# zhipeng-wei/Image-to-Video-I2V-attack

Measured on AMD Instinct MI355X. Metric: adversarial frames/sec (10-step I2V, ResNet-50 layer3, 32x224^2 clips), higher is better.
Workload: dtype f32

## Files before the change

image-to-video-i2v-attack_amd/csrc/i2v_conv_tile.h:

```cpp
#pragma once
#include "i2v_be.h"

#ifndef I2V_PROBE_T
struct I2VNoProbe {
    __device__ __forceinline__ void entry() {}
    __device__ __forceinline__ void loop_begin() {}
    __device__ __forceinline__ void loop_end(int ) {}
    __device__ __forceinline__ void exit(int ) {}
};
#define I2V_PROBE_T I2VNoProbe
#endif

#ifndef I2V_PRIO_LEVELS
#define I2V_PRIO_LEVELS 3
#endif
#ifndef I2V_DEEP
#define I2V_DEEP 1
#endif
#ifndef I2V_DEEP_STAGES
#define I2V_DEEP_STAGES 3
#endif
#ifndef I2V_BF3_STAGES
#define I2V_BF3_STAGES 2
#endif
#ifndef I2V_SMALL_WPE
#define I2V_SMALL_WPE 7
#endif
#ifndef I2V_PREF_WPE
#define I2V_PREF_WPE 6
#endif
#ifndef I2V_MID_WPE
#define I2V_MID_WPE 5
#endif
#ifndef I2V_TALL_WPE
#define I2V_TALL_WPE 6
#endif
#ifndef I2V_BIG_WPE
#define I2V_BIG_WPE 3
#endif

static constexpr int conv_waves_per_simd(int BD, int BP, bool PREF, bool hi, int MODE = 0) {
    return (BD == 64 && BP == 64) ? (PREF ? (I2V_DEEP && MODE == 1 && I2V_DEEP_STAGES > 3 ? 4  : I2V_PREF_WPE) : I2V_SMALL_WPE) : (BD == 128 && BP == 64) ? I2V_TALL_WPE : (BD == 32 && BP == 256) ? 4  : BD * BP == 8192 ? I2V_MID_WPE : BD * BP == 16384 ? I2V_BIG_WPE : (hi ? 8 : 1);
}
#define I2V_CONV_WPE __attribute__((amdgpu_waves_per_eu(conv_waves_per_simd(BD, BP, PREF, false, MODE), conv_waves_per_simd(BD, BP, PREF, true, MODE))))
static constexpr bool conv_deep(int MODE, bool PREF) { return I2V_DEEP && PREF && MODE == 1; }
template <int BD, int BP, int WD, bool MF16, int NST = 2, int CPB = 1, int BF3 = 0>
constexpr int conv_lds_floats() {
    constexpr int stage = NST * CPB * (I2V_KC * BP + (BF3 == 2 ? 0 : BF3 ? ((BD / 32) * 3 + 3) / 4 * 4 * 256 : I2V_KC * BD)), epi = WD * (MF16 ? 16 : 32) * BP;
    return stage > epi ? stage : epi;
}

template <int HWM>
constexpr int conv_halo_lds_floats() {
    constexpr int stage = 2 * I2V_KC * (64 + 64 + 2 * HWM + 2), epi = 64 * 64;
    return stage > epi ? stage : epi;
}

template <int BD, int BP, int WD, bool PREF, bool MF16, bool FUSE, typename PT>
__device__ __forceinline__ void conv_vec_rows(const PT& p, const int i, const int cd0, const int64_t px0, const float (*const Cs)[BP], const int t,
                                              const float4* const pre0, const unsigned* const pregw, float* const mid) {
    constexpr int FR = MF16 ? 16 : 32;
    const int lane = t & 63;
    const int HWg = p.Hg * p.Wg, HoWo = p.Ho * p.Wo;
    const int64_t P = (int64_t)p.N * HWg;
    (void)pre0; (void)pregw; (void)mid;
#ifdef I2V_NT_ALL
    const bool nt_store = true;
#else
    const bool nt_store = p.cfg > 0 && ((p.cfg - 1) & 128);
#endif
    constexpr int C4 = BP / 4, RSTEP = 1024 / BP, NQ = WD * FR / RSTEP;
    const int c4 = t % C4, rbase = t / C4;
    const int64_t pp = px0 + (int64_t)c4 * 4;
    const bool pok = pp < P;
    const int64_t n = pok ? fastdiv((unsigned)pp, p.dv_hw_m, p.dv_hw_s) : 0;
    const int64_t poff = pp - n * HWg;
    #pragma unroll
    for (int q = 0; q < NQ; ++q) {
        const int row = rbase + q * RSTEP;
        const int cd = cd0 + (row / FR) * (BD / WD) + i * FR + (row % FR);
        const bool valid = pok && cd < p.Cd;
        float4 v = make_float4(0.f, 0.f, 0.f, 0.f);
        if (valid) {
        v = *reinterpret_cast<const float4*>(&Cs[row][c4 * 4]);
        const int64_t o = (int64_t)cd * HoWo + poff;
        if (p.gate_scale) {
            const float4 m = *reinterpret_cast<const float4*>(p.mask + n * p.mask_nstride + o);
            const float gs = p.gate_scale[cd], gt = p.gate_shift[cd];
            if (!(fmaf(m.x, gs, gt) > 0.f)) v.x = 0.f;
            if (!(fmaf(m.y, gs, gt) > 0.f)) v.y = 0.f;
            if (!(fmaf(m.z, gs, gt) > 0.f)) v.z = 0.f;
            if (!(fmaf(m.w, gs, gt) > 0.f)) v.w = 0.f;
        }
        if (p.shift) { const float sh = p.shift[cd]; v.x += sh; v.y += sh; v.z += sh; v.w += sh; }
        if (PREF) {
            v.x += pre0[q].x; v.y += pre0[q].y; v.z += pre0[q].z; v.w += pre0[q].w;
        } else {
            if (p.add0 && p.add0_stride == 1) {
                const float4 a = *reinterpret_cast<const float4*>(p.add0 + n * p.add0_nstride + o);
                v.x += a.x; v.y += a.y; v.z += a.z; v.w += a.w;
            } else if (p.add0) {
                const int oh = (int)fastdiv((unsigned)poff, p.dv_wo_m, p.dv_wo_s), ow = (int)(poff - (int64_t)oh * p.Wo);
                if (!(oh & 1) && (oh >> 1) < p.add0_H) {
                    const float2 a = *reinterpret_cast<const float2*>(
                        p.add0 + n * p.add0_nstride + (int64_t)cd * p.add0_H * p.add0_W + (oh >> 1) * p.add0_W + (ow >> 1));
                    v.x += a.x; v.z += a.y;
                }
            }
        }
        if (p.add1) {
            const float4 a = *reinterpret_cast<const float4*>(p.add1 + n * p.add1_nstride + o);
            v.x += a.x; v.y += a.y; v.z += a.z; v.w += a.w;
        }
        if (p.relu) { v.x = fmaxf(v.x, 0.f); v.y = fmaxf(v.y, 0.f); v.z = fmaxf(v.z, 0.f); v.w = fmaxf(v.w, 0.f); }
        if (p.gate) {
            const unsigned w = PREF ? pregw[q] : p.gate[(int64_t)cd * p.gate_stride + ((p.gate_pix0 + pp) >> 5)];
            const unsigned g = w >> ((unsigned)(p.gate_pix0 + pp) & 31u);
            if (!(g & 1u)) v.x = 0.f;
            if (!(g & 2u)) v.y = 0.f;
            if (!(g & 4u)) v.z = 0.f;
            if (!(g & 8u)) v.w = 0.f;
        } else if (p.mask && !p.gate_scale) {
            const float4 m = *reinterpret_cast<const float4*>(p.mask + n * p.mask_nstride + o);
            if (!(m.x > 0.f)) v.x = 0.f;
            if (!(m.y > 0.f)) v.y = 0.f;
            if (!(m.z > 0.f)) v.z = 0.f;
            if (!(m.w > 0.f)) v.w = 0.f;
        }
        if constexpr (!FUSE) {
            if (nt_store) { typedef float nt4 __attribute__((ext_vector_type(4))); const nt4 w4 = {v.x, v.y, v.z, v.w};
                            __builtin_nontemporal_store(w4, reinterpret_cast<nt4*>(p.dst + n * p.dst_nstride + o)); }
            else *reinterpret_cast<float4*>(p.dst + n * p.dst_nstride + o) = v;
        }
        }
        if constexpr (FUSE)
            *reinterpret_cast<float4*>(mid + (cd - cd0) * BP + c4 * 4) = v;
        if (p.gate_out) {
            unsigned nib = valid ? ((v.x > 0.f ? 1u : 0u) | (v.y > 0.f ? 2u : 0u) | (v.z > 0.f ? 4u : 0u) | (v.w > 0.f ? 8u : 0u)) : 0u;
            nib <<= 4 * (lane & 7);
            nib |= (unsigned)__builtin_amdgcn_update_dpp(0, (int)nib, 0xB1, 0xF, 0xF, true);
            nib |= (unsigned)__builtin_amdgcn_update_dpp(0, (int)nib, 0x4E, 0xF, 0xF, true);
            nib |= (unsigned)__builtin_amdgcn_update_dpp(0, (int)nib, 0x141, 0xF, 0xF, true);
            if (valid && (lane & 7) == 0)
                p.gate_out[(int64_t)cd * p.gate_out_stride + ((p.gate_out_pix0 + pp) >> 5)] = nib;
        }
    }
}

#define I2V_FROW(r) (MF16 ? 4 * lk + (r) : ((r) & 3) + 8 * ((r) >> 2) + 4 * lk)
template <int BP, int WP, bool MF16, int TP, typename ACC>
__device__ __forceinline__ void conv_acc_to_rows(ACC (&acc)[TP], float (*const Cs)[BP]) {
    constexpr int FR = MF16 ? 16 : 32, NR = MF16 ? 4 : 16;
    const int lane = threadIdx.x & 63, wave = threadIdx.x >> 6;
    const int wd = wave / WP, wpx = wave % WP;
    const int l31 = MF16 ? (lane & 15) : (lane & 31), lk = MF16 ? (lane >> 4) : (lane >> 5);
    __syncthreads();
#pragma unroll
    for (int j = 0; j < TP; ++j)
#pragma unroll
        for (int r = 0; r < NR; ++r)
            Cs[wd * FR + I2V_FROW(r)][wpx * (BP / WP) + j * FR + l31] = acc[j][r];
    __syncthreads();
}
template <int BD, int BP, int WD, int WP, bool PREF, bool MF16, bool FUSE, typename ACC, typename PT>
__device__ __forceinline__ void conv_vec_epilogue(const PT& p, ACC (&acc)[BD / WD / (MF16 ? 16 : 32)][BP / WP / (MF16 ? 16 : 32)], const int cd0,
                                                  const int64_t px0, float* const smem, const float4* const pre0, const unsigned* const pregw,
                                                  float* const mid) {
    constexpr int FR = MF16 ? 16 : 32, TD = BD / WD / FR;
    const int t = threadIdx.x;
    float (*Cs)[BP] = reinterpret_cast<float (*)[BP]>(smem);
#pragma unroll
    for (int i = 0; i < TD; ++i) {
        conv_acc_to_rows<BP, WP, MF16>(acc[i], Cs);
        conv_vec_rows<BD, BP, WD, PREF, MF16, FUSE>(p, i, cd0, px0, Cs, t, pre0, pregw, mid);
    }
}
#undef I2V_FROW

__device__ __forceinline__ int conv_xcd_lid(const int bid, const int nwg) {
    const int q8 = nwg >> 3, r8 = nwg & 7, xcd = bid & 7;
    return (xcd < r8 ? xcd * (q8 + 1) : r8 * (q8 + 1) + (xcd - r8) * q8) + (bid >> 3);
}

template <int BD, int BP, int WD, int WP, int MODE, bool PREF, bool PRE = false, bool VID = false, bool MF16 = false, int HWM = 0, int CPB = 1, int FUSE = 0, int BF3 = 0>
__device__ __forceinline__ void conv_tile_loop(const I2VConvParams& p, const int cd0, const int64_t px0, const int nwg, float* const smem, I2V_PROBE_T& probe,
                                               const int probe_slot, const int prio_arg,
                                               typename std::conditional<MF16, f32x4, f32x16>::type (&acc)[BD / WD / (MF16 ? 16 : 32)][BP / WP / (MF16 ? 16 : 32)],
                                               float4 (&pre0)[PREF ? WD * (MF16 ? 16 : 32) / (1024 / BP) : 1], unsigned (&pregw)[PREF ? WD * (MF16 ? 16 : 32) / (1024 / BP) : 1]) {
#if defined(__HIP_DEVICE_COMPILE__)
    constexpr int KC = I2V_KC;
    constexpr int FR = MF16 ? 16 : 32;
    constexpr int NR = MF16 ? 4 : 16;
    constexpr int TD = BD / WD / FR, TP = BP / WP / FR;
    static_assert(!(MF16 && (PRE || PREF)), "no pre-activation / prefetch variants of the 16x16 tile");
    constexpr bool DEEP = conv_deep(MODE, PREF) || (BF3 == 1 && I2V_BF3_STAGES > 2) || BF3 == 3;
    constexpr int NST = BF3 == 3 ? 3 : BF3 == 1 ? I2V_BF3_STAGES : DEEP ? I2V_DEEP_STAGES : 2, AHEAD = NST - 1;
    constexpr bool HALO = MODE == 5;
    constexpr int HS = HALO ? BP + 2 * HWM + 2 : 1, HQ = (HS + 63) / 64;
    static_assert(!HALO || (HWM > 0 && BD == 64 && BP == 64 && !PREF && !PRE && !VID && !MF16), "halo staging: the plain 64x64 image tile only");
    static_assert(CPB == 1 || (!HALO && !DEEP && !PREF && !PRE && MODE != 4 && MODE != 0), "several chunks per barrier: the plain pointwise / tap-uniform loops only");
    constexpr int KB = CPB * KC;
    static_assert(!BF3 || (!MF16 && !PRE && !PREF && !HALO && (MODE == 1 || MODE == 2) && FUSE == 0 && BD % 32 == 0), "split-bf16 K loop: the plain pointwise / tap-uniform tiles");
    constexpr int AF = BF3 == 2 ? 0 : BF3 ? CPB * (((BD / 32) * 3 + 3) / 4 * 4) * 256 : KB * BD;
    float (*As)[KB][BD] = reinterpret_cast<float (*)[KB][BD]>(smem);
    float* const As3 = smem;
    float (*Bs)[KB][BP] = reinterpret_cast<float (*)[KB][BP]>(smem + NST * AF);

    const int t = threadIdx.x, lane = t & 63, wave = t >> 6;
    const int wd = wave / WP, wpx = wave % WP;

    const int HWg = p.Hg * p.Wg;
    const int64_t P = (int64_t)p.N * HWg;

    constexpr bool PW = MODE == 1;
    constexpr bool QUAD = MODE == 4;
    typedef __attribute__((address_space(3))) void* lds_ptr_t;
    constexpr unsigned OOB = 0x80000000u;
    const int wv = __builtin_amdgcn_readfirstlane(wave);
    const __amdgpu_buffer_rsrc_t rs_w = BF3 ? __builtin_amdgcn_make_buffer_rsrc((void*)p.wp3, 0, (p.Kpad / KC) * (p.Cdpad / 32) * 3072, 0x00020000)
                                            : __builtin_amdgcn_make_buffer_rsrc((void*)p.wp, 0, p.Kpad * p.Cdpad * 4, 0x00020000);
    constexpr unsigned XB = QUAD ? 64u : 0u;
    const __amdgpu_buffer_rsrc_t rs_x = __builtin_amdgcn_make_buffer_rsrc((void*)((const char*)p.src - XB), 0, p.src_span_bytes + 2 * XB, 0x00020000);
    constexpr int NA = BF3 == 2 ? 0 : BF3 ? (BD / 32) * 3 : KC * BD / 256, NAQ = (NA + 3) / 4;
    constexpr int BPER = (PW || QUAD) ? 256 : 64;
    constexpr int NB = HALO ? 0 : KC * BP / BPER, NBQ = (NB + 3) / 4;
    const int bcol = PW ? (lane * 4) % BP : (BP >= 64 ? ((wave * 64) % BP) + lane : lane % BP);
    const int64_t ppix = px0 + bcol;
    const bool pvalid = ppix < P;
    const int64_t pn = pvalid ? fastdiv((unsigned)ppix, p.dv_hw_m, p.dv_hw_s) : 0;
    const int prem = (int)(ppix - pn * HWg);
    const int HWs = p.Hs * p.Ws;
    int h0 = 0, w0 = 0, t0 = 0;
    int64_t pns = pn;
    if (VID) {
        const int64_t clip = fastdiv((unsigned)pn, p.dv_t_m, p.dv_t_s);
        t0 = (int)(pn - clip * p.Tg) * p.st;
        pns = clip * p.Ts + t0;
    }
    const int nstr = (int)p.src_nstride;
    unsigned xoff;
    if (PW) xoff = (unsigned)((pns * p.src_nstride + prem) * 4);
    else {
        const int gi = (int)fastdiv((unsigned)prem, p.dv_w_m, p.dv_w_s), gj = prem - gi * p.Wg;
        h0 = gi * p.sh; w0 = gj * p.sw;
        xoff = (unsigned)((pns * p.src_nstride + (int64_t)h0 * p.Ws + w0) * 4) + XB;
    }
    if (!pvalid) xoff = OOB;
    unsigned aoff[NAQ ? NAQ : 1];
#pragma unroll
    for (int q = 0; q < NAQ; ++q) {
        const int f = (wave + 4 * q) * 256 + lane * 4;
        aoff[q] = BF3 ? (unsigned)(((cd0 / 32) * 3 + wave + 4 * q) * 1024 + lane * 16) : (unsigned)(((f / BD) * p.Cdpad + f % BD + cd0) * 4);
    }
    unsigned boff[PW ? NBQ : 1];
    if (PW) {
#pragma unroll
        for (int q = 0; q < NBQ; ++q) boff[q] = pvalid ? xoff + (unsigned)((((wave + 4 * q) * 256 + lane * 4) / BP) * HWs * 4) : OOB;
    }

#define I2V_ISSUE_PIECE(j_, k0_, buf_, vb_) I2V_ISSUE_PIECE_SUB(j_, k0_, buf_, vb_, 0)
#define I2V_ISSUE_PIECE_SUB(j_, k0_, buf_, vb_, sub_)                                                     \
    {                                                                                                     \
        constexpr int jj = (j_);                                                                          \
        const int k0 = (k0_);                                                                             \
        if constexpr (jj < NAQ) {                                                                         \
            const int ins = wv + 4 * jj;                                                                  \
            if constexpr (BF3) {    \
                __builtin_amdgcn_raw_ptr_buffer_load_lds(rs_w, (lds_ptr_t)(As3 + (buf_) * AF + (sub_) * (AF / CPB) + ins * 256), 16, ins < NA ? aoff[jj] : OOB, \
                                                         (k0 / KC) * (p.Cdpad / 32) * 3072, 0, 0);       \
            } else if (NA % 4 == 0 || ins < NA) {                                                         \
                if constexpr (false)                                                                      \
                    ;                                                                                     \
                else                                                                                      \
                    __builtin_amdgcn_raw_ptr_buffer_load_lds(rs_w, (lds_ptr_t)(&As[buf_][(sub_) * KC][0] + ins * 256), 16, aoff[jj],  \
                                                             k0 * p.Cdpad * 4, 0, 0);                     \
            }                                                                                             \
        } else {                                                                                          \
            constexpr int q = jj - NAQ;                                                                   \
            const int ins = wv + 4 * q;                                                                   \
            float* const bbuf = &Bs[buf_][(sub_) * KC][0];                                                \
            if (NB % 4 == 0 || ins < NB) {                                                                \
                if constexpr (PW) {                                                                       \
                    unsigned v = boff[q];                                                                 \
                    if (k0 + KC > p.K)             \
                        v = (k0 + ((wave + 4 * q) * 256 + lane * 4) / BP < p.K) ? v : OOB;                \
                    __builtin_amdgcn_raw_ptr_buffer_load_lds(rs_x, (lds_ptr_t)(bbuf + ins * 256), 16, v,         \
                                                             k0 * HWs * 4, 0, 0);                         \
                } else if constexpr (QUAD) {                                                              \
                     \
                    const I2VKEntry e = load_kentry(p.ktab, k0 + 4 * ((ins * 64) / BP));                  \
                    const int hs = h0 + e.dh, dtk = VID ? (e.valid >> 1) : 0;                             \
                    const bool ok = pvalid && (unsigned)hs < (unsigned)p.Hs && (!VID || (unsigned)(t0 + dtk) < (unsigned)p.Ts); \
                    const unsigned v = ok ? xoff + (unsigned)((e.chan_off + dtk * nstr + e.dh * p.Ws + e.dw) * 4) : OOB; \
                    __builtin_amdgcn_raw_ptr_buffer_load_lds(rs_x, (lds_ptr_t)(bbuf + ins * 256), 16, v, 0, 0, 0); \
                } else if constexpr (MODE == 2) {                                                         \
                    __builtin_amdgcn_raw_ptr_buffer_load_lds(rs_x, (lds_ptr_t)(bbuf + ins * 64), 4, vb_,         \
                                                             ((ins * 64) / BP) * HWs * 4, 0, 0);          \
                } else {                                                                                  \
                    const I2VKEntry e = load_kentry(p.ktab, k0 + (ins * 64) / BP);                        \
                    const int hs = h0 + e.dh, ws = w0 + e.dw, dtk = VID ? (e.valid >> 1) : 0;             \
                    const bool ok = pvalid && (e.valid & 1) && (unsigned)hs < (unsigned)p.Hs &&           \
                                    (unsigned)ws < (unsigned)p.Ws && (!VID || (unsigned)(t0 + dtk) < (unsigned)p.Ts); \
                    const unsigned v = ok ? xoff + (unsigned)((e.chan_off + dtk * nstr + e.dh * p.Ws + e.dw) * 4) : OOB; \
                    __builtin_amdgcn_raw_ptr_buffer_load_lds(rs_x, (lds_ptr_t)(bbuf + ins * 64), 4, v, 0, 0, 0); \
                }                                                                                         \
            }                                                                                             \
        }                                                                                                 \
    }
#define I2V_CHUNK_VB(e_)                                                                                  \
    ([&]() -> unsigned {                                                                                  \
        const int hs = h0 + (e_).dh, ws = w0 + (e_).dw, dtk = VID ? ((e_).valid >> 1) : 0;                \
        const bool ok = pvalid && (unsigned)hs < (unsigned)p.Hs && (unsigned)ws < (unsigned)p.Ws &&       \
                        (!VID || (unsigned)(t0 + dtk) < (unsigned)p.Ts);                                  \
        return ok ? xoff + (unsigned)(((e_).chan_off + dtk * nstr + (e_).dh * p.Ws + (e_).dw) * 4) : OOB; \
    }())

    constexpr int E_C4 = BP / 4, E_RSTEP = 1024 / BP, E_NQ = WD * FR / E_RSTEP;
    static_assert(!PREF || TD == 1, "PREF needs a single epilogue pass");
    static_assert(!PREF || E_NQ == WD * (MF16 ? 16 : 32) / (1024 / BP), "pre0 / pregw (the caller's): one entry per row a lane owns");
    if (PREF) {
        const int e_c4 = t % E_C4, e_rbase = t / E_C4;
        const int64_t e_pp = px0 + (int64_t)e_c4 * 4;
        const bool e_ok = e_pp < P;
        const int64_t e_n = e_ok ? fastdiv((unsigned)e_pp, p.dv_hw_m, p.dv_hw_s) : 0;
        const int64_t e_poff = e_pp - e_n * HWg;
        const int e_HoWo = p.Ho * p.Wo;
#pragma unroll
// ... 294 lines not shown
#pragma unroll
                            for (int pl = 0; pl < 3; ++pl) wa[i][pl] = wcur[sub][i][pl];
                    } else {
                        const float* const abase = As3 + buf * AF + sub * (AF / CPB) + lane * 4;
#pragma unroll
                        for (int i = 0; i < TD; ++i)
#pragma unroll
                            for (int pl = 0; pl < 3; ++pl)
                                wa[i][pl] = __builtin_bit_cast(bf8, *reinterpret_cast<const f4*>(abase + ((wd * TD + i) * 3 + pl) * 256));
                    }
#pragma unroll
                    for (int j = 0; j < TP; ++j) {
                        float x[8];
#pragma unroll
                        for (int e = 0; e < 8; ++e) x[e] = Bs[buf][sub * KC + 8 * lk + e][wpx * (BP / WP) + j * FR + l31];
                        unsigned q1[4], q2[4], q3[4];
#pragma unroll
                        for (int e = 0; e < 4; ++e) split2(x[2 * e], x[2 * e + 1], q1[e], q2[e], q3[e]);
                        typedef unsigned u4 __attribute__((ext_vector_type(4)));
                        xb[j][0] = __builtin_bit_cast(bf8, (u4){q1[0], q1[1], q1[2], q1[3]});
                        xb[j][1] = __builtin_bit_cast(bf8, (u4){q2[0], q2[1], q2[2], q2[3]});
                        xb[j][2] = __builtin_bit_cast(bf8, (u4){q3[0], q3[1], q3[2], q3[3]});
                    }
                    constexpr int TW[6] = {2, 1, 0, 1, 0, 0}, TX[6] = {0, 1, 2, 0, 1, 0};
                    [&]<int... M>(std::integer_sequence<int, M...>) {
                        (([&] {
                            constexpr int m = M, term = m / (TD * TP), ij = m % (TD * TP), i = ij / TP, j = ij % TP;
                            acc[i][j] = __builtin_amdgcn_mfma_f32_32x32x16_bf16(wa[i][TW[term]], xb[j][TX[term]], acc[i][j], 0, 0, 0);
                            if constexpr (MORE) {
                                constexpr int jp = sub * 6 * TD * TP + m;
                                if constexpr (jp < CPB * NL) {
                                    constexpr int sb2 = jp / NL;
                                    I2V_ISSUE_PIECE_SUB(jp % NL, ((c + AHEAD) * CPB + sb2) * KC, (buf + AHEAD) % NST, vb[sb2], sb2);
                                }
                            }
                        }()), ...);
                    }(std::make_integer_sequence<int, 6 * TD * TP>{});
                }()), ...);
            }(std::make_integer_sequence<int, CPB>{});
            if constexpr (BF3 == 2 && MORE) {
#pragma unroll
                for (int sb = 0; sb < CPB; ++sb)
#pragma unroll
                    for (int i = 0; i < TD; ++i)
#pragma unroll
                        for (int pl = 0; pl < 3; ++pl) wcur[sb][i][pl] = wnxt[sb][i][pl];
            }
            return;
        }
        float fa[2][TD], fb[2][TP];
        auto read_frags = [&](const int s, const int set) {
#pragma unroll
            for (int i = 0; i < TD; ++i) fa[set][i] = As[buf][KR * s + lk][wd * (BD / WD) + i * FR + l31];
            if constexpr (QUAD) {
                const float* const bq = &Bs[buf][0][0];
#pragma unroll
                for (int j = 0; j < TP; ++j) {
                    const int px = wpx * (BP / WP) + j * FR + l31;
                    const int qd = MF16 ? s : (s >> 1), el = MF16 ? lk : 2 * (s & 1) + lk;
                    const float v = bq[(qd * BP + px) * 4 + el];
                    const bool m = ((qd & 1) && p.quad == 2) ? qok[j][1][MF16 ? 0 : (s & 1)] : qok[j][0][MF16 ? 0 : (s & 1)];
                    fb[set][j] = m ? v : 0.f;
                }
            } else {
#pragma unroll
                for (int j = 0; j < TP; ++j) fb[set][j] = Bs[buf][KR * s + lk][wpx * (BP / WP) + j * FR + l31];
            }
        };
        read_frags(0, 0);
        [&]<int... S>(std::integer_sequence<int, S...>) {
            (([&] {
                constexpr int s = S, set = S & 1;
                if constexpr (s + 1 < CPB * KS) read_frags(s + 1, set ^ 1);
                __builtin_amdgcn_sched_barrier(0);
                if constexpr (PRE) {
                    typedef const __attribute__((address_space(4))) float* cfp;
                    const int kr = c * KB + 2 * s;
                    const float sc = lk ? ((cfp)p.pre_scale)[kr + 1] : ((cfp)p.pre_scale)[kr];
                    const float sh = lk ? ((cfp)p.pre_shift)[kr + 1] : ((cfp)p.pre_shift)[kr];
#pragma unroll
                    for (int j = 0; j < TP; ++j) fb[set][j] = fmaxf(fmaf(fb[set][j], sc, sh), 0.f);
                }
#pragma unroll
                for (int i = 0; i < TD; ++i)
#pragma unroll
                    for (int j = 0; j < TP; ++j) {
                        if constexpr (MF16) acc[i][j] = __builtin_amdgcn_mfma_f32_16x16x4f32(fa[set][i], fb[set][j], acc[i][j], 0, 0, 0);
                        else acc[i][j] = __builtin_amdgcn_mfma_f32_32x32x2f32(fa[set][i], fb[set][j], acc[i][j], 0, 0, 0);
                    }
                if constexpr (MORE) {
                    [&]<int... Q>(std::integer_sequence<int, Q...>) {
                        (([&] {
                            constexpr int jp = s * PPS + Q;
                            if constexpr (jp < CPB * NL) {
                                constexpr int sub = jp / NL;
                                I2V_ISSUE_PIECE_SUB(jp % NL, ((c + AHEAD) * CPB + sub) * KC, DEEP ? (buf + AHEAD) % NST : (buf ^ 1), vb[sub], sub);
                            }
                        }()), ...);
                    }(std::make_integer_sequence<int, PPS>{});
                }
            }()), ...);
        }(std::make_integer_sequence<int, CPB * KS>{});
    };
    if constexpr (BF3 == 3) {
        asm volatile("s_waitcnt vmcnt(0)" ::: "memory");
        __builtin_amdgcn_s_barrier();
        const int l31_ = lane & 31, lk_ = lane >> 5;
#pragma unroll
        for (int j = 0; j < TP_; ++j) {
            float x[8];
#pragma unroll
            for (int e = 0; e < 8; ++e) x[e] = Bs[0][8 * lk_ + e][(wave % WP) * (BP / WP) + j * 32 + l31_];
            bf3_split_frag(x, xcur[j]);
        }
    }
    if constexpr (!HALO) {
        int c = 0, buf = 0;
        for (; c + AHEAD < nsuper; ++c) { chunk_body(c, buf, std::true_type{}); buf = buf + 1 == NST ? 0 : buf + 1; }
        for (; c < nsuper; ++c) { chunk_body(c, buf, std::false_type{}); buf = buf + 1 == NST ? 0 : buf + 1; }
    }
#undef I2V_ISSUE_PIECE
#undef I2V_ISSUE_PIECE_SUB
#undef I2V_CHUNK_VB
    if (prio_hi > 0) __builtin_amdgcn_s_setprio(0);
    probe.loop_end(probe_slot);
#endif
}

template <int BD, int BP, int WD, int WP, int MODE, bool PREF, bool PRE = false, bool VID = false, bool MF16 = false, int HWM = 0, int CPB = 1, int FUSE = 0, int BF3 = 0>
__device__ __forceinline__ void conv_tile(const I2VConvParams& p, const int n_cd_tiles, const int bid, const int nwg, const int64_t px_base,
                                          float* const smem, I2V_PROBE_T& probe, const int probe_slot, const int prio_arg = I2V_PRIO_LEVELS,
                                          float* const mid = nullptr) {
#if defined(__HIP_DEVICE_COMPILE__)
    constexpr int FR = MF16 ? 16 : 32, NR = MF16 ? 4 : 16, TD = BD / WD / FR, TP = BP / WP / FR;
    const int lid = conv_xcd_lid(bid, nwg);
    const int cd_tile = lid % n_cd_tiles;
    const int64_t px0 = px_base + (int64_t)(lid / n_cd_tiles) * BP;
    const int cd0 = cd_tile * BD;

    constexpr int E_NQ = WD * FR / (1024 / BP);
    float4 pre0[PREF ? E_NQ : 1];
    unsigned pregw[PREF ? E_NQ : 1];
    typename std::conditional<MF16, f32x4, f32x16>::type acc[TD][TP];
    conv_tile_loop<BD, BP, WD, WP, MODE, PREF, PRE, VID, MF16, HWM, CPB, FUSE, BF3>(p, cd0, px0, nwg, smem, probe, probe_slot, prio_arg, acc, pre0, pregw);

    const int lane = threadIdx.x & 63, wave = threadIdx.x >> 6;
    const int wd = wave / WP, wpx = wave % WP;
    const int l31 = MF16 ? (lane & 15) : (lane & 31), lk = MF16 ? (lane >> 4) : (lane >> 5);
    const int HWg = p.Hg * p.Wg;
    const int64_t P = (int64_t)p.N * HWg;
#define I2V_FROW(r) (MF16 ? 4 * lk + (r) : ((r) & 3) + 8 * ((r) >> 2) + 4 * lk)
    const int HoWo = p.Ho * p.Wo;
    if (p.vec_epilogue) {
        conv_vec_epilogue<BD, BP, WD, WP, PREF, MF16, FUSE != 0>(p, acc, cd0, px0, smem, pre0, pregw, mid);
        return;
    }
    if (p.blk > 1 || (VID && p.blkt > 1)) {
        const int bb = p.blk * p.blk, Creal = p.Cd / ((VID ? p.blkt : 1) * bb);
#pragma unroll
        for (int j = 0; j < TP; ++j) {
            const int64_t pp = px0 + wpx * (BP / WP) + j * FR + l31;
            if (pp >= P) continue;
            const int64_t ng = fastdiv((unsigned)pp, p.dv_hw_m, p.dv_hw_s);
            const int rem = (int)(pp - ng * HWg);
            const int gi = (int)fastdiv((unsigned)rem, p.dv_w_m, p.dv_w_s), gj = rem - gi * p.Wg;
            const int64_t clip = VID ? fastdiv((unsigned)ng, p.dv_t_m, p.dv_t_s) : ng;
            const int otb = VID ? (int)(ng - clip * p.Tg) * p.ost + p.ot0 : 0;
#pragma unroll
            for (int i = 0; i < TD; ++i)
#pragma unroll
                for (int r = 0; r < NR; ++r) {
                    const int cd = cd0 + wd * (BD / WD) + i * FR + I2V_FROW(r);
                    if (cd >= p.Cd) continue;
                    const int cls3 = cd / Creal, c = cd - cls3 * Creal;
                    const int ct = VID ? cls3 / bb : 0, cls = cls3 - ct * bb;
                    const int oh = gi * p.osh + cls / p.blk + p.oh0, ow = gj * p.osw + cls % p.blk + p.ow0;
                    if (oh >= p.Ho || ow >= p.Wo || (VID && otb + ct * p.oct >= p.To)) continue;
                    const int64_t n = VID ? clip * p.To + otb + ct * p.oct : ng;
                    const int64_t o = (int64_t)c * HoWo + oh * p.Wo + ow;
                    float v = acc[i][j][r];
                    if (p.shift) v += p.shift[c];
                    if (p.add1) v += p.add1[n * p.add1_nstride + o];
                    if (p.relu) v = fmaxf(v, 0.f);
                    if (p.mask && !(p.mask[n * p.mask_nstride + o] > 0.f)) v = 0.f;
                    p.dst[n * p.dst_nstride + o] = v;
                }
        }
        return;
    }
#pragma unroll
    for (int j = 0; j < TP; ++j) {
        const int64_t pp = px0 + wpx * (BP / WP) + j * FR + l31;
        const bool pin = pp < P;
        const int64_t ng = pin ? fastdiv((unsigned)pp, p.dv_hw_m, p.dv_hw_s) : 0;
        const int rem = (int)(pin ? pp - ng * HWg : 0);
        const int gi = (int)fastdiv((unsigned)rem, p.dv_w_m, p.dv_w_s), gj = rem - gi * p.Wg;
        const int oh = gi * p.osh + p.oh0, ow = gj * p.osw + p.ow0;
        bool ok = pin && oh < p.Ho && ow < p.Wo;
        int64_t n = ng;
        if (VID) {
            const int64_t clip = fastdiv((unsigned)ng, p.dv_t_m, p.dv_t_s);
            const int ot = (int)(ng - clip * p.Tg) * p.ost + p.ot0;
            if (ot >= p.To) ok = false;
            n = clip * p.To + ot;
        }
        const int opix = oh * p.Wo + ow;
        float* dstn = p.dst + n * p.dst_nstride + opix;
        const float* a0 = nullptr; int a0_plane = HoWo;
        if (p.add0 && ok) {
            if (p.add0_stride == 1) a0 = p.add0 + n * p.add0_nstride + opix;
            else {
                const int s = p.add0_stride, qh = oh / s, qw = ow / s;
                if (qh * s == oh && qw * s == ow && qh < p.add0_H && qw < p.add0_W) {
                    a0 = p.add0 + n * p.add0_nstride + qh * p.add0_W + qw;
                    a0_plane = p.add0_H * p.add0_W;
                }
            }
        }
        const float* a1 = p.add1 ? p.add1 + n * p.add1_nstride + opix : nullptr;
        const float* mk = p.mask ? p.mask + n * p.mask_nstride + opix : nullptr;
        const int64_t gidx = (int64_t)p.gate_pix0 + n * HoWo + opix;
#pragma unroll
        for (int i = 0; i < TD; ++i) {
#pragma unroll
            for (int r = 0; r < NR; ++r) {
                const int cd = cd0 + wd * (BD / WD) + i * FR + I2V_FROW(r);
                const bool okc = ok && cd < p.Cd;
                float v = 0.f;
                if (okc) {
                    v = acc[i][j][r];
                    if (p.gate_scale && !(fmaf(mk[(int64_t)cd * HoWo], p.gate_scale[cd], p.gate_shift[cd]) > 0.f)) v = 0.f;
                    if (p.shift) v += p.shift[cd];
                    if (a0) v += a0[(int64_t)cd * a0_plane];
                    if (a1) v += a1[(int64_t)cd * HoWo];
                    if (p.relu) v = fmaxf(v, 0.f);
                    if (p.gate) { if (!((p.gate[(int64_t)cd * p.gate_stride + (gidx >> 5)] >> (gidx & 31)) & 1u)) v = 0.f; }
                    else if (mk && !p.gate_scale && !(mk[(int64_t)cd * HoWo] > 0.f)) v = 0.f;
                    dstn[(int64_t)cd * HoWo] = v;
                }
                if (p.gate_out) {
                    const unsigned long long bal = __ballot(okc && v > 0.f);
                    if (l31 == 0 && pin && cd < p.Cd) {
                        const int64_t bit0 = (int64_t)p.gate_out_pix0 + pp;
                        if constexpr (MF16)
                            reinterpret_cast<uint16_t*>(p.gate_out + (int64_t)cd * p.gate_out_stride)[bit0 >> 4] = (uint16_t)(bal >> (16 * lk));
                        else
                            p.gate_out[(int64_t)cd * p.gate_out_stride + (bit0 >> 5)] = (unsigned)(bal >> (32 * lk));
                    }
                }
            }
        }
    }
#undef I2V_FROW
#endif
}

template <int BD, int BP, int WD, int WP, int MODE, bool PREF, bool PRE = false, bool VID = false, bool MF16 = false>
__global__ void __launch_bounds__(256) I2V_CONV_WPE conv_igemm(const I2VConvParams p, const int n_cd_tiles) {
    __shared__ __attribute__((aligned(16))) float smem[conv_lds_floats<BD, BP, WD, MF16, conv_deep(MODE, PREF) ? I2V_DEEP_STAGES : 2>()];
    I2V_PROBE_T probe;
    probe.entry();
    conv_tile<BD, BP, WD, WP, MODE, PREF, PRE, VID, MF16>(p, n_cd_tiles, blockIdx.x, gridDim.x, 0, smem, probe, blockIdx.x);
    probe.exit(blockIdx.x);
}

template <int HWM>
__global__ void __launch_bounds__(256) __attribute__((amdgpu_waves_per_eu(HWM <= 14 ? I2V_SMALL_WPE : (HWM <= 28 ? 6 : 5), HWM <= 14 ? I2V_SMALL_WPE : (HWM <= 28 ? 6 : 5))))
conv_igemm_halo(const I2VConvParams p, const int n_cd_tiles) {
    __shared__ __attribute__((aligned(16))) float smem[conv_halo_lds_floats<HWM>()];
    I2V_PROBE_T probe;
    probe.entry();
    conv_tile<64, 64, 2, 2, 5, false, false, false, false, HWM>(p, n_cd_tiles, blockIdx.x, gridDim.x, 0, smem, probe, blockIdx.x);
    probe.exit(blockIdx.x);
}

#ifndef I2V_DC_WPE
#define I2V_DC_WPE 5
#endif
template <int MODE, int CPB>
__global__ void __launch_bounds__(256) __attribute__((amdgpu_waves_per_eu(I2V_DC_WPE, I2V_DC_WPE)))
conv_igemm_dc(const I2VConvParams p, const int n_cd_tiles) {
    __shared__ __attribute__((aligned(16))) float smem[conv_lds_floats<64, 64, 2, false, 2, CPB>()];
    I2V_PROBE_T probe;
    probe.entry();
    conv_tile<64, 64, 2, 2, MODE, false, false, false, false, 0, CPB>(p, n_cd_tiles, blockIdx.x, gridDim.x, 0, smem, probe, blockIdx.x);
    probe.exit(blockIdx.x);
}


template <int MODE>
__global__ void __launch_bounds__(256) __attribute__((amdgpu_waves_per_eu(I2V_SMALL_WPE, I2V_SMALL_WPE)))
conv_igemm_tail(const I2VConvParams p, const int n_cd_a, const int nA, const int n_cd_b, const int64_t px_base_b) {
    constexpr int LA = conv_lds_floats<64, 64, 2, false>(), LB = conv_lds_floats<16, 64, 1, true>();
    __shared__ __attribute__((aligned(16))) float smem[LA > LB ? LA : LB];
    I2V_PROBE_T probe;
    probe.entry();
    const int slot = (int)blockIdx.x < nA ? (int)blockIdx.x : 65536 + (int)blockIdx.x - nA;
    if ((int)blockIdx.x < nA) conv_tile<64, 64, 2, 2, MODE, false, false, false, false>(p, n_cd_a, blockIdx.x, nA, 0, smem, probe, slot, I2V_PRIO_LEVELS > 2 ? 2 : I2V_PRIO_LEVELS);
    else {
        if (I2V_PRIO_LEVELS > 0) __builtin_amdgcn_s_setprio(3);
        conv_tile<16, 64, 1, 4, MODE, false, false, false, true>(p, n_cd_b, (int)blockIdx.x - nA, (int)gridDim.x - nA, px_base_b, smem, probe, slot, 0);
        if (I2V_PRIO_LEVELS > 0) __builtin_amdgcn_s_setprio(0);
    }
    probe.exit(slot);
}
```

Measured before the change: 755.2.

## Batch vectorized epilogue rows into groups to overlap global loads

Restructures the vectorized conv epilogue so each thread handles several output rows at once. It issues all side-input loads (shift, residual add, mask, gate words) for the group before any arithmetic, so memory latency overlaps across rows. Group size adapts to how many inputs are active, with a fast path for fully in-bounds tiles chosen by a wave ballot. Large tile configurations are forced to the serial per-row path to limit register pressure. The cost is more live registers and code size, which could lower occupancy or cause spills.

```diff
diff --git a/image-to-video-i2v-attack_amd/csrc/i2v_conv_tile.h b/image-to-video-i2v-attack_amd/csrc/i2v_conv_tile.h
--- a/image-to-video-i2v-attack_amd/csrc/i2v_conv_tile.h
+++ b/image-to-video-i2v-attack_amd/csrc/i2v_conv_tile.h
@@ -56,7 +56,20 @@
     return stage > epi ? stage : epi;
 }
 
-template <int BD, int BP, int WD, bool PREF, bool MF16, bool FUSE, typename PT>
+#ifndef I2V_EPI_GROUP
+#define I2V_EPI_GROUP 0
+#endif
+template <int BD, int BP, int WD, bool MF16, bool FUSE>
+constexpr int conv_epi_group(const bool heavy, const int cap) {
+    constexpr int NQ = WD * (MF16 ? 16 : 32) / (1024 / BP);
+    int g = I2V_EPI_GROUP ? I2V_EPI_GROUP : BP == 256 ? 4 : 2;
+    if (heavy && g > 1) g /= 2;
+    if (cap < 0) g = 1;
+    else if (cap && g > cap) g = cap;
+    return FUSE ? 1 : NQ < g ? NQ : g;
+}
+
+template <int BD, int BP, int WD, bool PREF, bool MF16, bool FUSE, int GCAP = 0, typename PT>
 __device__ __forceinline__ void conv_vec_rows(const PT& p, const int i, const int cd0, const int64_t px0, const float (*const Cs)[BP], const int t,
                                               const float4* const pre0, const unsigned* const pregw, float* const mid) {
     constexpr int FR = MF16 ? 16 : 32;
@@ -75,75 +88,194 @@
     const bool pok = pp < P;
     const int64_t n = pok ? fastdiv((unsigned)pp, p.dv_hw_m, p.dv_hw_s) : 0;
     const int64_t poff = pp - n * HWg;
+    constexpr bool SERIAL = GCAP < 0;
+    constexpr int GL = conv_epi_group<BD, BP, WD, MF16, FUSE>(false, GCAP), GH = conv_epi_group<BD, BP, WD, MF16, FUSE>(true, GCAP);
+    static_assert(NQ % GL == 0 && NQ % GH == 0, "a thread's rows split into whole groups");
+    const bool a0_dense = !PREF && p.add0 && p.add0_stride == 1, a0_compact = !PREF && p.add0 && p.add0_stride != 1;
+    const bool need_mask = p.gate_scale || (!p.gate && p.mask);
+    static_assert(FR % RSTEP == 0, "a thread's rows keep their place inside a fragment");
+    const int cdl = cd0 + i * FR + rbase;
+    const int64_t ol = (int64_t)cdl * HoWo + poff;
+    auto dq = [](const int q) constexpr { return ((q * RSTEP) / FR) * (BD / WD) + (q * RSTEP) % FR; };
+    auto group = [&]<int G, bool HEAVY, bool ALL>(std::integral_constant<int, G>, std::bool_constant<HEAVY>, std::bool_constant<ALL>, const int q0) __attribute__((always_inline)) {
+        constexpr int GX = HEAVY ? G : 1;
+        int cd[G];
+        bool valid[G];
+        int64_t ro[G];
+        float4 v[G], a0[G], mk[GX], a1[GX];
+        float sh[G], gs[GX], gt[GX];
+        unsigned gw[G];
+        bool a0c_ok = false;
+        int a0c_off = 0;
+#pragma unroll
+        for (int g = 0; g < G; ++g) {
+            const int row = rbase + (q0 + g) * RSTEP;
+            cd[g] = cdl + dq(q0 + g);
+            valid[g] = ALL || (pok && cd[g] < p.Cd);
+            ro[g] = (int64_t)dq(q0 + g) * HoWo;
+            v[g] = make_float4(0.f, 0.f, 0.f, 0.f);
+            if (valid[g]) v[g] = *reinterpret_cast<const float4*>(&Cs[row][c4 * 4]);
+        }
+        const auto ld_gs = [&]() __attribute__((always_inline)) {
+            if (HEAVY && p.gate_scale) {
     #pragma unroll
-    for (int q = 0; q < NQ; ++q) {
-        const int row = rbase + q * RSTEP;
-        const int cd = cd0 + (row / FR) * (BD / WD) + i * FR + (row % FR);
-        const bool valid = pok && cd < p.Cd;
-        float4 v = make_float4(0.f, 0.f, 0.f, 0.f);
-        if (valid) {
-        v = *reinterpret_cast<const float4*>(&Cs[row][c4 * 4]);
-        const int64_t o = (int64_t)cd * HoWo + poff;
-        if (p.gate_scale) {
-            const float4 m = *reinterpret_cast<const float4*>(p.mask + n * p.mask_nstride + o);
-            const float gs = p.gate_scale[cd], gt = p.gate_shift[cd];
-            if (!(fmaf(m.x, gs, gt) > 0.f)) v.x = 0.f;
-            if (!(fmaf(m.y, gs, gt) > 0.f)) v.y = 0.f;
-            if (!(fmaf(m.z, gs, gt) > 0.f)) v.z = 0.f;
-            if (!(fmaf(m.w, gs, gt) > 0.f)) v.w = 0.f;
-        }
-        if (p.shift) { const float sh = p.shift[cd]; v.x += sh; v.y += sh; v.z += sh; v.w += sh; }
+                for (int g = 0; g < G; ++g)
+                    if (valid[g]) { gs[g] = p.gate_scale[cd[g]]; gt[g] = p.gate_shift[cd[g]]; }
+            }
+        };
+        const auto ld_mk = [&]() __attribute__((always_inline)) {
+            if (HEAVY && need_mask) {
+    #pragma unroll
+                for (int g = 0; g < G; ++g)
+                    if (valid[g]) mk[g] = *reinterpret_cast<const float4*>(p.mask + (n * p.mask_nstride + ol) + ro[g]);
+            }
+        };
+        const auto ld_sh = [&]() __attribute__((always_inline)) {
+            if (p.shift) {
+    #pragma unroll
+                for (int g = 0; g < G; ++g)
+                    if (valid[g]) sh[g] = p.shift[cd[g]];
+            }
+        };
+        const auto ld_a0 = [&]() __attribute__((always_inline)) {
+            if (a0_dense) {
+    #pragma unroll
+                for (int g = 0; g < G; ++g)
+                    if (valid[g]) a0[g] = *reinterpret_cast<const float4*>(p.add0 + (n * p.add0_nstride + ol) + ro[g]);
+            } else if (a0_compact) {
+                if (pok) {
+                    const int oh = (int)fastdiv((unsigned)poff, p.dv_wo_m, p.dv_wo_s), ow = (int)(poff - (int64_t)oh * p.Wo);
+                    a0c_ok = !(oh & 1) && (oh >> 1) < p.add0_H;
+                    a0c_off = (oh >> 1) * p.add0_W + (ow >> 1);
+                }
+    #pragma unroll
+                for (int g = 0; g < G; ++g)
+                    if (a0c_ok && valid[g]) {
+                        const float2 a = *reinterpret_cast<const float2*>(p.add0 + (n * p.add0_nstride + (int64_t)cdl * p.add0_H * p.add0_W + a0c_off) + (int64_t)dq(q0 + g) * p.add0_H * p.add0_W);
+                        a0[g].x = a.x; a0[g].y = a.y;
+                    }
+            }
+        };
+        const auto ld_a1 = [&]() __attribute__((always_inline)) {
+            if (HEAVY && p.add1) {
+    #pragma unroll
+                for (int g = 0; g < G; ++g)
+                    if (valid[g]) a1[g] = *reinterpret_cast<const float4*>(p.add1 + (n * p.add1_nstride + ol) + ro[g]);
+            }
+        };
+        const auto ld_gw = [&]() __attribute__((always_inline)) {
+            if (!PREF && p.gate) {
+                const int64_t gword = (p.gate_pix0 + pp) >> 5;
+    #pragma unroll
+                for (int g = 0; g < G; ++g)
+                    if (valid[g]) gw[g] = p.gate[((int64_t)cdl * p.gate_stride + gword) + (int64_t)dq(q0 + g) * p.gate_stride];
+            }
+        };
+        if constexpr (!SERIAL) { ld_gs(); ld_mk(); ld_sh(); ld_a0(); ld_a1(); ld_gw(); }
+        if (HEAVY && p.gate_scale) {
+            if constexpr (SERIAL) { ld_gs(); ld_mk(); }
+#pragma unroll
+            for (int g = 0; g < G; ++g)
+                if (valid[g]) {
+                    if (!(fmaf(mk[g].x, gs[g], gt[g]) > 0.f)) v[g].x = 0.f;
+                    if (!(fmaf(mk[g].y, gs[g], gt[g]) > 0.f)) v[g].y = 0.f;
+                    if (!(fmaf(mk[g].z, gs[g], gt[g]) > 0.f)) v[g].z = 0.f;
+                    if (!(fmaf(mk[g].w, gs[g], gt[g]) > 0.f)) v[g].w = 0.f;
+                }
+        }
+        if (p.shift) {
+            if constexpr (SERIAL) ld_sh();
+#pragma unroll
+            for (int g = 0; g < G; ++g)
+                if (valid[g]) { v[g].x += sh[g]; v[g].y += sh[g]; v[g].z += sh[g]; v[g].w += sh[g]; }
+        }
+        if constexpr (SERIAL) ld_a0();
         if (PREF) {
-            v.x += pre0[q].x; v.y += pre0[q].y; v.z += pre0[q].z; v.w += pre0[q].w;
+#pragma unroll
+            for (int g = 0; g < G; ++g)
+                if (valid[g]) { v[g].x += pre0[q0 + g].x; v[g].y += pre0[q0 + g].y; v[g].z += pre0[q0 + g].z; v[g].w += pre0[q0 + g].w; }
+        } else if (a0_dense) {
+#pragma unroll
+            for (int g = 0; g < G; ++g)
+                if (valid[g]) { v[g].x += a0[g].x; v[g].y += a0[g].y; v[g].z += a0[g].z; v[g].w += a0[g].w; }
+        } else if (a0_compact) {
+#pragma unroll
+            for (int g = 0; g < G; ++g)
+                if (a0c_ok && valid[g]) { v[g].x += a0[g].x; v[g].z += a0[g].y; }
+        }
+        if (HEAVY && p.add1) {
+            if constexpr (SERIAL) ld_a1();
+#pragma unroll
+            for (int g = 0; g < G; ++g)
+                if (valid[g]) { v[g].x += a1[g].x; v[g].y += a1[g].y; v[g].z += a1[g].z; v[g].w += a1[g].w; }
+        }
+        if (p.relu) {
+#pragma unroll
+            for (int g = 0; g < G; ++g)
+                if (valid[g]) { v[g].x = fmaxf(v[g].x, 0.f); v[g].y = fmaxf(v[g].y, 0.f); v[g].z = fmaxf(v[g].z, 0.f); v[g].w = fmaxf(v[g].w, 0.f); }
+        }
+        if (p.gate) {
+            if constexpr (SERIAL) ld_gw();
+            const unsigned gbit = (unsigned)(p.gate_pix0 + pp) & 31u;
+#pragma unroll
+            for (int g = 0; g < G; ++g)
+                if (valid[g]) {
+                    const unsigned b = (PREF ? pregw[q0 + g] : gw[g]) >> gbit;
+                    if (!(b & 1u)) v[g].x = 0.f;
+                    if (!(b & 2u)) v[g].y = 0.f;
+                    if (!(b & 4u)) v[g].z = 0.f;
+                    if (!(b & 8u)) v[g].w = 0.f;
+                }
+        } else if (HEAVY && p.mask && !p.gate_scale) {
+            if constexpr (SERIAL) ld_mk();
+#pragma unroll
+            for (int g = 0; g < G; ++g)
+                if (valid[g]) {
+                    if (!(mk[g].x > 0.f)) v[g].x = 0.f;
+                    if (!(mk[g].y > 0.f)) v[g].y = 0.f;
+                    if (!(mk[g].z > 0.f)) v[g].z = 0.f;
+                    if (!(mk[g].w > 0.f)) v[g].w = 0.f;
+                }
+        }
+        if constexpr (!FUSE) {
+            if (nt_store) {
+                typedef float nt4 __attribute__((ext_vector_type(4)));
+#pragma unroll
+                for (int g = 0; g < G; ++g)
+                    if (valid[g]) { const nt4 w4 = {v[g].x, v[g].y, v[g].z, v[g].w};
+                                    __builtin_nontemporal_store(w4, reinterpret_cast<nt4*>(p.dst + (n * p.dst_nstride + ol) + ro[g])); }
+            } else {
+#pragma unroll
+                for (int g = 0; g < G; ++g)
+                    if (valid[g]) *reinterpret_cast<float4*>(p.dst + (n * p.dst_nstride + ol) + ro[g]) = v[g];
+            }
         } else {
-            if (p.add0 && p.add0_stride == 1) {
-                const float4 a = *reinterpret_cast<const float4*>(p.add0 + n * p.add0_nstride + o);
-                v.x += a.x; v.y += a.y; v.z += a.z; v.w += a.w;
-            } else if (p.add0) {
-                const int oh = (int)fastdiv((unsigned)poff, p.dv_wo_m, p.dv_wo_s), ow = (int)(poff - (int64_t)oh * p.Wo);
-                if (!(oh & 1) && (oh >> 1) < p.add0_H) {
-                    const float2 a = *reinterpret_cast<const float2*>(
-                        p.add0 + n * p.add0_nstride + (int64_t)cd * p.add0_H * p.add0_W + (oh >> 1) * p.add0_W + (ow >> 1));
-                    v.x += a.x; v.z += a.y;
-                }
-            }
-        }
-        if (p.add1) {
-            const float4 a = *reinterpret_cast<const float4*>(p.add1 + n * p.add1_nstride + o);
-            v.x += a.x; v.y += a.y; v.z += a.z; v.w += a.w;
-        }
-        if (p.relu) { v.x = fmaxf(v.x, 0.f); v.y = fmaxf(v.y, 0.f); v.z = fmaxf(v.z, 0.f); v.w = fmaxf(v.w, 0.f); }
-        if (p.gate) {
-            const unsigned w = PREF ? pregw[q] : p.gate[(int64_t)cd * p.gate_stride + ((p.gate_pix0 + pp) >> 5)];
-            const unsigned g = w >> ((unsigned)(p.gate_pix0 + pp) & 31u);
-            if (!(g & 1u)) v.x = 0.f;
-            if (!(g & 2u)) v.y = 0.f;
-            if (!(g & 4u)) v.z = 0.f;
-            if (!(g & 8u)) v.w = 0.f;
-        } else if (p.mask && !p.gate_scale) {
-            const float4 m = *reinterpret_cast<const float4*>(p.mask + n * p.mask_nstride + o);
-            if (!(m.x > 0.f)) v.x = 0.f;
-            if (!(m.y > 0.f)) v.y = 0.f;
-            if (!(m.z > 0.f)) v.z = 0.f;
-            if (!(m.w > 0.f)) v.w = 0.f;
-        }
-        if constexpr (!FUSE) {
-            if (nt_store) { typedef float nt4 __attribute__((ext_vector_type(4))); const nt4 w4 = {v.x, v.y, v.z, v.w};
-                            __builtin_nontemporal_store(w4, reinterpret_cast<nt4*>(p.dst + n * p.dst_nstride + o)); }
-            else *reinterpret_cast<float4*>(p.dst + n * p.dst_nstride + o) = v;
-        }
-        }
-        if constexpr (FUSE)
-            *reinterpret_cast<float4*>(mid + (cd - cd0) * BP + c4 * 4) = v;
+#pragma unroll
+            for (int g = 0; g < G; ++g) *reinterpret_cast<float4*>(mid + (cd[g] - cd0) * BP + c4 * 4) = v[g];
+        }
         if (p.gate_out) {
-            unsigned nib = valid ? ((v.x > 0.f ? 1u : 0u) | (v.y > 0.f ? 2u : 0u) | (v.z > 0.f ? 4u : 0u) | (v.w > 0.f ? 8u : 0u)) : 0u;
-            nib <<= 4 * (lane & 7);
-            nib |= (unsigned)__builtin_amdgcn_update_dpp(0, (int)nib, 0xB1, 0xF, 0xF, true);
-            nib |= (unsigned)__builtin_amdgcn_update_dpp(0, (int)nib, 0x4E, 0xF, 0xF, true);
-            nib |= (unsigned)__builtin_amdgcn_update_dpp(0, (int)nib, 0x141, 0xF, 0xF, true);
-            if (valid && (lane & 7) == 0)
-                p.gate_out[(int64_t)cd * p.gate_out_stride + ((p.gate_out_pix0 + pp) >> 5)] = nib;
-        }
+#pragma unroll
+            for (int g = 0; g < G; ++g) {
+                unsigned nib = valid[g] ? ((v[g].x > 0.f ? 1u : 0u) | (v[g].y > 0.f ? 2u : 0u) | (v[g].z > 0.f ? 4u : 0u) | (v[g].w > 0.f ? 8u : 0u)) : 0u;
+                nib <<= 4 * (lane & 7);
+                nib |= (unsigned)__builtin_amdgcn_update_dpp(0, (int)nib, 0xB1, 0xF, 0xF, true);
+                nib |= (unsigned)__builtin_amdgcn_update_dpp(0, (int)nib, 0x4E, 0xF, 0xF, true);
+                nib |= (unsigned)__builtin_amdgcn_update_dpp(0, (int)nib, 0x141, 0xF, 0xF, true);
+                if (valid[g] && (lane & 7) == 0)
+                    p.gate_out[((int64_t)cdl * p.gate_out_stride + ((p.gate_out_pix0 + pp) >> 5)) + (int64_t)dq(q0 + g) * p.gate_out_stride] = nib;
+            }
+        }
+    };
+    const bool all_in = pok && cdl + dq(NQ - 1) < p.Cd;
+    if ((GL == 1 && GH == 1) || __builtin_amdgcn_ballot_w64(!all_in) != 0) {
+#pragma unroll
+        for (int q0 = 0; q0 < NQ; ++q0) group(std::integral_constant<int, 1>{}, std::true_type{}, std::false_type{}, q0);
+    } else if (need_mask || p.add1) {
+#pragma unroll
+        for (int q0 = 0; q0 < NQ; q0 += GH) group(std::integral_constant<int, GH>{}, std::true_type{}, std::true_type{}, q0);
+    } else {
+#pragma unroll
+        for (int q0 = 0; q0 < NQ; q0 += GL) group(std::integral_constant<int, GL>{}, std::false_type{}, std::true_type{}, q0);
     }
 }
 
@@ -162,7 +294,7 @@
             Cs[wd * FR + I2V_FROW(r)][wpx * (BP / WP) + j * FR + l31] = acc[j][r];
     __syncthreads();
 }
-template <int BD, int BP, int WD, int WP, bool PREF, bool MF16, bool FUSE, typename ACC, typename PT>
+template <int BD, int BP, int WD, int WP, bool PREF, bool MF16, bool FUSE, int GCAP = 0, typename ACC, typename PT>
 __device__ __forceinline__ void conv_vec_epilogue(const PT& p, ACC (&acc)[BD / WD / (MF16 ? 16 : 32)][BP / WP / (MF16 ? 16 : 32)], const int cd0,
                                                   const int64_t px0, float* const smem, const float4* const pre0, const unsigned* const pregw,
                                                   float* const mid) {
@@ -172,7 +304,7 @@
 #pragma unroll
     for (int i = 0; i < TD; ++i) {
         conv_acc_to_rows<BP, WP, MF16>(acc[i], Cs);
-        conv_vec_rows<BD, BP, WD, PREF, MF16, FUSE>(p, i, cd0, px0, Cs, t, pre0, pregw, mid);
+        conv_vec_rows<BD, BP, WD, PREF, MF16, FUSE, GCAP>(p, i, cd0, px0, Cs, t, pre0, pregw, mid);
     }
 }
 #undef I2V_FROW
@@ -773,7 +905,7 @@
 #define I2V_FROW(r) (MF16 ? 4 * lk + (r) : ((r) & 3) + 8 * ((r) >> 2) + 4 * lk)
     const int HoWo = p.Ho * p.Wo;
     if (p.vec_epilogue) {
-        conv_vec_epilogue<BD, BP, WD, WP, PREF, MF16, FUSE != 0>(p, acc, cd0, px0, smem, pre0, pregw, mid);
+        conv_vec_epilogue<BD, BP, WD, WP, PREF, MF16, FUSE != 0, ((MODE == 4 && BD == 128 && BP == 64) || BD * BP == 16384) ? -1 : 0>(p, acc, cd0, px0, smem, pre0, pregw, mid);
         return;
     }
     if (p.blk > 1 || (VID && p.blkt > 1)) {
```

Result: no change. 761.8, median of 6 (+0.9%).
